# raznem/spp-rl

Measured on AMD Instinct MI355X. Metric: env-steps/sec (rollout+update) SPP-SAC Hopper-v2, higher is better.
Workload: dtype fp32

## Files before the change

### spp-rl_amd/csrc/common.h

```cpp
#pragma once
#include <hip/hip_runtime.h>
#include <stdint.h>

#include <string>

#ifndef SPP_BF16_TWO_TILES
#define SPP_BF16_TWO_TILES 0
#endif
#ifndef SPP_BF16_FUSE3
#define SPP_BF16_FUSE3 0
#endif

typedef float f32x16 __attribute__((ext_vector_type(16)));
typedef float f32x4 __attribute__((ext_vector_type(4)));

namespace spp {

constexpr int kWave = 64;
constexpr int kTile = 32;
constexpr int kHidden = 256;

void set_error(const char* fmt, ...);
const char* get_error();

#define SPP_CHECK_HIP(expr)                                                        \
  do {                                                                             \
    hipError_t e_ = (expr);                                                        \
    if (e_ != hipSuccess) {                                                        \
      ::spp::set_error("%s:%d %s -> %s", __FILE__, __LINE__, #expr, hipGetErrorString(e_)); \
      return SPP_E_HIP;                                                            \
    }                                                                              \
  } while (0)

#define SPP_REQUIRE(cond, code, ...)        \
  do {                                      \
    if (!(cond)) {                          \
      ::spp::set_error(__VA_ARGS__);        \
      return code;                          \
    }                                       \
  } while (0)

inline int64_t round_up(int64_t x, int64_t m) { return (x + m - 1) / m * m; }
inline int cdiv(int64_t x, int64_t m) { return (int)((x + m - 1) / m); }
// ... 82 lines not shown
```

### spp-rl_amd/csrc/mlp.h

```cpp
#pragma once
#include "common.h"

namespace spp {
#define SPP_XLANE_SYNC() asm volatile("" ::: "memory")


#ifdef SPP_PROF
__device__ unsigned long long g_tprof[64];
__shared__ unsigned long long s_tprof[4][32];
__shared__ unsigned long long s_tlast[4];
#ifdef SPP_PROF_DRAIN
#define SPP_TP_DRAIN() asm volatile("s_waitcnt vmcnt(0) lgkmcnt(0)" ::: "memory")
#else
#define SPP_TP_DRAIN()
#endif
#define SPP_TP_INIT()                                                            \
  {                                                                              \
    const int w_ = threadIdx.x >> 6;                                             \
    if ((threadIdx.x & 63) < 32 && w_ < 4) s_tprof[w_][threadIdx.x & 63] = 0;    \
    if ((threadIdx.x & 63) == 0 && w_ < 4) s_tlast[w_] = clock64();              \
  }
#define SPP_TP(k)                                                                \
  {                                                                              \
    __builtin_amdgcn_sched_barrier(0);                                           \
// ... 133 lines not shown
  for (int b = 0; b < NBI; ++b) {
    if (q < base + rv_get(RV, b)) return q - base;
    base += rv_get(RV, b);
  }
  return 0;
}

__device__ __forceinline__ constexpr int ru(int r) { return (r & 3) + 8 * (r >> 2); }

__device__ __forceinline__ f32x16 bias_tile(const float* biasL, int ob, int h) {
  f32x16 acc;
  const float4* b4 = reinterpret_cast<const float4*>(biasL + 32 * ob + 4 * h);
#pragma unroll
  for (int k = 0; k < 4; ++k) {
    const float4 v = b4[2 * k];
    acc[4 * k + 0] = v.x;
    acc[4 * k + 1] = v.y;
    acc[4 * k + 2] = v.z;
    acc[4 * k + 3] = v.w;
  }
  return acc;
}

typedef __amdgpu_buffer_rsrc_t rsrc_t;
__device__ __forceinline__ rsrc_t rsrc_n(const void* p, int nbytes) {
  return __builtin_amdgcn_make_buffer_rsrc(const_cast<void*>(p), (short)0, nbytes, 0x00020000);
}
__device__ __forceinline__ rsrc_t rsrc(const void* p) { return rsrc_n(p, 0x7fffffff); }
__device__ __forceinline__ float4 wfrag(rsrc_t w, uint32_t lane16, int off) {
  asm volatile("" : "+s"(off));
  return __builtin_bit_cast(float4, __builtin_amdgcn_raw_buffer_load_b128(w, lane16, off, 0));
}

template <int NBI, uint64_t RV, bool BIAS, typename Epi>
__device__ __forceinline__ void dense_impl(const float4* __restrict__ Wf, int NBO, const f32x16 (&in)[NBI],
                                           const float* biasL, Epi&& epi) {
  constexpr int NQ = rv_total(RV, NBI);
  static_assert(NQ > 0, "empty layer");
  constexpr int CH = chunk_of(NQ);
  constexpr int NC = NQ / CH;
  static_assert(NQ % CH == 0, "chunking");
  const int lane = lane_id();
  const int h = lane >> 5;
  const rsrc_t wr = rsrc(Wf);
  const uint32_t l16 = 16u * lane;
  constexpr int OBSTRIDE = NBI * 4 * 64 * 16;
  float4 cur[CH];
  static_for<0, CH>([&](auto I) {
    constexpr int q = decltype(I)::value;
    cur[q] = wfrag(wr, l16, (q_ib(RV, NBI, q) * 4 + q_rq(RV, NBI, q)) * 1024);
  });
  auto chain = [&](int ob) {
    f32x16 acc;
    if constexpr (BIAS) acc = bias_tile(biasL, ob, h);
    else acc = zero16();
    const int obn = ob + 1 < NBO ? ob + 1 : ob;
    static_for<0, NC>([&](auto C) {
      constexpr int c = decltype(C)::value;
      constexpr int nc = (c + 1 < NC) ? c + 1 : 0;
      const int wn = ((c + 1 < NC) ? ob : obn) * OBSTRIDE;
      float4 nxt[CH];
      static_for<0, CH>([&](auto I) {
        constexpr int q = nc * CH + decltype(I)::value;
        nxt[decltype(I)::value] = wfrag(wr, l16, wn + (q_ib(RV, NBI, q) * 4 + q_rq(RV, NBI, q)) * 1024);
      });
      static_for<0, CH>([&](auto I) {
        constexpr int i = decltype(I)::value;
        constexpr int q = c * CH + i;
        constexpr int ib = q_ib(RV, NBI, q);
        constexpr int rq = q_rq(RV, NBI, q);
        acc = mfma(cur[i].x, in[ib][4 * rq + 0], acc);
        acc = mfma(cur[i].y, in[ib][4 * rq + 1], acc);
        acc = mfma(cur[i].z, in[ib][4 * rq + 2], acc);
        acc = mfma(cur[i].w, in[ib][4 * rq + 3], acc);
      });
#pragma unroll
      for (int i = 0; i < CH; ++i) cur[i] = nxt[i];
    });
    return acc;
  };
  SPP_TPD(23);
  f32x16 prev = chain(0);
#pragma unroll 1
  for (int ob = 1; ob < NBO; ++ob) {
    const f32x16 acc = chain(ob);
    epi(ob - 1, prev);
    prev = acc;
  }
  SPP_TPD(24);
  epi(NBO - 1, prev);
  SPP_TPD(25);
}

constexpr int cgcd(int a, int b) { return b ? cgcd(b, a % b) : a; }

template <int NBO, bool BIAS, typename Epi>
__device__ __forceinline__ void dense_lds_impl(const float4* __restrict__ Wf, const float* img, const float* biasL,
                                               Epi&& epi) {
  constexpr int NQ = NBO * 4;
  constexpr int CH = 4;
  constexpr int NCI = NQ / CH;
  constexpr int D = 4;
  constexpr int U = NCI * D / cgcd(NCI, D);
  constexpr int IBU = U / NCI;
  constexpr int G = 8 * NCI;
  static_assert(8 % IBU == 0, "input blocks per iteration");
  constexpr int NIT = 8 / IBU;
  const int lane = lane_id();
  const int h = lane >> 5;
  const float* l = img + 4 * h * 32 + (lane & 31);
  const rsrc_t wr = rsrc(Wf);
  const uint32_t l16 = 16u * lane;
  f32x16 acc[NBO];
  static_for<0, NBO>([&](auto O) {
    if constexpr (BIAS) acc[O] = bias_tile(biasL, O, h);
    else acc[O] = zero16();
  });
  float4 ring[D][CH];
  static_for<0, D - 1>([&](auto I) {
    static_for<0, CH>([&](auto J) { ring[I][J] = wfrag(wr, l16, ((int)I * CH + (int)J) * 1024); });
  });
  f32x16 xin[IBU];
  static_for<0, IBU>([&](auto K) {
// ... 45 lines not shown
  return __builtin_amdgcn_mfma_f32_32x32x16_bf16(a, b, c, 0, 0, 0);
}
__device__ __forceinline__ bf16x8 frag16(float4 v) { return __builtin_bit_cast(bf16x8, v); }
template <int S>
__device__ __forceinline__ bf16x8 to_bf16x8(const f32x16& t) {
  bf16x8 r;
#pragma unroll
  for (int j = 0; j < 8; ++j) r[j] = (__bf16)t[8 * S + j];
  return r;
}
constexpr int st_get(uint64_t RV, int ib) { return (rv_get(RV, ib) + 1) / 2; }
constexpr int st_total(uint64_t RV, int nb) {
  int t = 0;
  for (int ib = 0; ib < nb; ++ib) t += st_get(RV, ib);
  return t;
}
constexpr int st_ib(uint64_t RV, int NBI, int q) {
  int base = 0;
  for (int b = 0; b < NBI; ++b) {
    if (q < base + st_get(RV, b)) return b;
    base += st_get(RV, b);
  }
  return NBI - 1;
}
constexpr int st_s(uint64_t RV, int NBI, int q) {
  int base = 0;
  for (int b = 0; b < NBI; ++b) {
    if (q < base + st_get(RV, b)) return q - base;
    base += st_get(RV, b);
  }
  return 0;
}

template <int NBI, uint64_t RV, bool BIAS, typename Epi>
__device__ __forceinline__ void dense16_impl(const float4* __restrict__ Wf, int NBO, const f32x16 (&in)[NBI],
                                             const float* biasL, Epi&& epi) {
  constexpr int NS = st_total(RV, NBI);
  static_assert(NS > 0, "empty layer");
  const int lane = lane_id();
  const int h = lane >> 5;
  const rsrc_t wr = rsrc(Wf);
  const uint32_t l16 = 16u * lane;
  constexpr int OBSTRIDE = NBI * 2 * 64 * 16;
  bf16x8 bin[NS];
  static_for<0, NS>([&](auto Q) {
    constexpr int q = Q;
    bin[q] = to_bf16x8<st_s(RV, NBI, q)>(in[st_ib(RV, NBI, q)]);
  });
  float4 cur[NS];
  static_for<0, NS>([&](auto Q) {
    constexpr int q = Q;
    cur[q] = wfrag(wr, l16, (st_ib(RV, NBI, q) * 2 + st_s(RV, NBI, q)) * 1024);
  });
  auto chain = [&](int ob) {
    f32x16 acc;
    if constexpr (BIAS) acc = bias_tile(biasL, ob, h);
    else acc = zero16();
    const int wn = (ob + 1 < NBO ? ob + 1 : ob) * OBSTRIDE;
    float4 nxt[NS];
    static_for<0, NS>([&](auto Q) {
      constexpr int q = Q;
      nxt[q] = wfrag(wr, l16, wn + (st_ib(RV, NBI, q) * 2 + st_s(RV, NBI, q)) * 1024);
    });
    static_for<0, NS>([&](auto Q) { acc = mfma16(frag16(cur[(int)Q]), bin[(int)Q], acc); });
#pragma unroll
    for (int q = 0; q < NS; ++q) cur[q] = nxt[q];
    return acc;
  };
  f32x16 prev = chain(0);
#pragma unroll 1
  for (int ob = 1; ob < NBO; ++ob) {
    const f32x16 acc = chain(ob);
    epi(ob - 1, prev);
    prev = acc;
  }
  epi(NBO - 1, prev);
}

template <int NBO, bool BIAS, typename Epi>
__device__ __forceinline__ void dense16_lds_impl(const float4* __restrict__ Wf, const float* img, const float* biasL,
                                                 Epi&& epi) {
  const int lane = lane_id();
  const int h = lane >> 5;
  const float* l = img + 4 * h * 32 + (lane & 31);
  const rsrc_t wr = rsrc(Wf);
  const uint32_t l16 = 16u * lane;
  f32x16 acc[NBO];
  static_for<0, NBO>([&](auto O) {
    if constexpr (BIAS) acc[O] = bias_tile(biasL, O, h);
    else acc[O] = zero16();
  });
  float4 fr[2][2 * NBO];
  static_for<0, 2 * NBO>([&](auto J) { fr[0][J] = wfrag(wr, l16, (int)J * 1024); });
  f32x16 x;
#pragma unroll
  for (int r = 0; r < 16; ++r) x[r] = l[ru(r) * 32];
  static_for<0, 8>([&](auto IB) {
    constexpr int ib = IB;
    const bf16x8 b0 = to_bf16x8<0>(x), b1 = to_bf16x8<1>(x);
    if constexpr (ib + 1 < 8) {
      static_for<0, 2 * NBO>([&](auto J) {
        fr[(ib + 1) & 1][J] = wfrag(wr, l16, ((ib + 1) * NBO * 2 + (int)J) * 1024);
      });
    }
    __builtin_amdgcn_sched_barrier(0);
    static_for<0, NBO>([&](auto O) {
      constexpr int ob = O;
      acc[ob] = mfma16(frag16(fr[ib & 1][2 * ob]), b0, acc[ob]);
      acc[ob] = mfma16(frag16(fr[ib & 1][2 * ob + 1]), b1, acc[ob]);
    });
    if constexpr (ib + 1 < 8) {
#pragma unroll
      for (int r = 0; r < 16; ++r) x[r] = l[(32 * (ib + 1) + ru(r)) * 32];
    }
  });
  static_for<0, NBO>([&](auto O) { epi(IC<(int)O>{}, acc[O]); });
}

template <int NBI, uint64_t RV, bool BF = false, typename Epi>
__device__ __forceinline__ void dense(const float4* __restrict__ Wf, int NBO, const f32x16 (&in)[NBI],
                                      const float* biasL, Epi&& epi) {
  if constexpr (BF) dense16_impl<NBI, RV, true>(Wf, NBO, in, biasL, static_cast<Epi&&>(epi));
  else dense_impl<NBI, RV, true>(Wf, NBO, in, biasL, static_cast<Epi&&>(epi));
}
template <int NBI, uint64_t RV, bool BF = false, typename Epi>
__device__ __forceinline__ void dense(const float4* __restrict__ Wf, int NBO, const f32x16 (&in)[NBI], decltype(nullptr),
                                      Epi&& epi) {
  if constexpr (BF) dense16_impl<NBI, RV, false>(Wf, NBO, in, nullptr, static_cast<Epi&&>(epi));
  else dense_impl<NBI, RV, false>(Wf, NBO, in, nullptr, static_cast<Epi&&>(epi));
}
template <int NBO, bool BF = false, typename Epi>
__device__ __forceinline__ void dense_lds(const float4* __restrict__ Wf, const float* img, const float* biasL,
                                          Epi&& epi) {
  if constexpr (BF) dense16_lds_impl<NBO, true>(Wf, img, biasL, static_cast<Epi&&>(epi));
  else dense_lds_impl<NBO, true>(Wf, img, biasL, static_cast<Epi&&>(epi));
}
template <int NBO, bool BF = false, typename Epi>
__device__ __forceinline__ void dense_lds(const float4* __restrict__ Wf, const float* img, decltype(nullptr),
                                          Epi&& epi) {
  if constexpr (BF) dense16_lds_impl<NBO, false>(Wf, img, nullptr, static_cast<Epi&&>(epi));
  else dense_lds_impl<NBO, false>(Wf, img, nullptr, static_cast<Epi&&>(epi));
}


#ifndef SPP_OPST_AUX
#define SPP_OPST_AUX 2
#endif
#ifndef SPP_STREAM_LD_AUX
#define SPP_STREAM_LD_AUX 0
#endif

__device__ __forceinline__ int lane_off(int ld, int b) { return 4 * (lane_id() >> 5) * ld + b; }

template <int NB>
__device__ __forceinline__ void lds_load(f32x16 (&t)[NB], const float* lds) {
  const int lane = lane_id();
  const float* l = lds + 4 * (lane >> 5) * 32 + (lane & 31);
#pragma unroll
  for (int ib = 0; ib < NB; ++ib)
#pragma unroll
    for (int r = 0; r < 16; ++r) t[ib][r] = l[(32 * ib + ru(r)) * 32];
}
// ... 57 lines not shown
```

### spp-rl_amd/csrc/sac.hip

```cpp
#pragma once
#include "sac_kernels.h"

namespace spp {

constexpr float kLog2 = 0.69314718055994530942f;
constexpr float kLogSqrt2Pi = 0.91893853320467274178f;

template <int OB_, int AOUT_, int AC_, bool ACMC_, bool BF_ = false>
struct Cfg {
  static constexpr int OB = OB_, AOUT = AOUT_, AC = AC_;
  static constexpr bool ACMC = ACMC_;
  static constexpr bool BF = BF_;
  static constexpr bool F3 = !BF_ || SPP_BF16_FUSE3;
  static constexpr int NB_OB = blocks_of(OB);
  static constexpr int NB_AOUT = blocks_of(AOUT);
  static constexpr int NB_H2 = blocks_of(2 * AOUT);
  static constexpr int NB_PAIR = (AOUT + 15) / 16;
  static constexpr int CA = ACMC ? AC : AOUT;
  static constexpr int NB_CA = blocks_of(CA);
  static constexpr int NB_CIN = NB_OB + NB_CA;
  static constexpr int NB_ACMIN = NB_OB + NB_AOUT;
  static constexpr uint64_t RV_X = rv_nat(OB, NB_OB);
  static constexpr uint64_t RV_H = rv_nat(256, 8);
  static constexpr uint64_t RV_CIN = rv_cat(OB, NB_OB, CA, NB_CA);
  static constexpr uint64_t RV_ACMIN = rv_cat(OB, NB_OB, AOUT, NB_AOUT);
  static constexpr uint64_t RV_Z1 = rv_nat(64, 2);
  static constexpr uint64_t RV_Z2 = rv_nat(32, 1);
  static constexpr uint64_t RV_AC = rv_nat(AC, 1);
  static constexpr uint64_t RV_CA = rv_nat(CA, NB_CA);
  static constexpr uint64_t RV_PAIR = rv_pair(AOUT, NB_PAIR);
  static_assert(AC <= 32, "env action dim <= 32");
  static_assert(2 * AOUT <= 256 && OB + AOUT <= 256, "dims");
};

constexpr int kWavesPerWG = 4;

constexpr int kLdsPerWave = 256 * 32;
constexpr int kSmallRow = 192;

__device__ __forceinline__ void load_table(const SacArgs& p, float* tbl) {
  for (int s = 0; s < p.nseg; ++s) {
    const TabSeg g = p.seg[s];
    for (int i = threadIdx.x; i < g.npad; i += blockDim.x) tbl[g.off + i] = i < g.n ? g.src[i] : 0.f;
  }
  __syncthreads();
}
__device__ __forceinline__ float tval(const float* t, int ob, int q, int h4) { return t[32 * ob + ru(q) + h4]; }
__device__ __forceinline__ void tvals(const float* t, int ob, int h4, float (&v)[16]) {
  const float4* p = reinterpret_cast<const float4*>(t + 32 * ob + h4);
#pragma unroll
  for (int k = 0; k < 4; ++k) {
    const float4 x = p[2 * k];
    v[4 * k + 0] = x.x;
    v[4 * k + 1] = x.y;
    v[4 * k + 2] = x.z;
    v[4 * k + 3] = x.w;
  }
}

__device__ __forceinline__ void setbits(uint64_t& lo, uint64_t& hi, int ob, uint32_t bits) {
  if (ob < 4) lo |= (uint64_t)bits << (16 * ob);
  else hi |= (uint64_t)bits << (16 * (ob - 4));
  asm volatile("" : "+v"(lo), "+v"(hi));
}
__device__ __forceinline__ bool getbit(uint64_t lo, uint64_t hi, int ob, int q) {
  const uint64_t w = ob < 4 ? (lo >> (16 * ob)) : (hi >> (16 * (ob - 4)));
// ... 121 lines not shown
  uint32_t vo, vp;
  float *bl, *sl;
  float* pl;
};
__device__ __forceinline__ Lane make_lane(float* big, float* small, const float* tbl, int ld, int b) {
  Lane L;
  L.img = big;
  L.tbl = tbl;
  int lane = lane_id();
  asm volatile("" : "+v"(lane));
  int ld4 = 4 * ld;
  asm volatile("" : "+s"(ld4));
  L.h = lane >> 5;
  L.s = lane & 31;
  L.h4 = 4 * L.h;
  L.ld4 = ld4;
  L.b = b;
  L.vo = (uint32_t)(L.h4 * ld4 + 4 * b);
  L.vp = (uint32_t)(8 * L.h * ld4 + 4 * b);
  L.bl = big + L.h4 * 32 + L.s;
  L.sl = small + L.h4 * 32 + L.s;
  L.pl = big + 8 * L.h * 32 + L.s;
  return L;
}

template <class C, bool ST, int NBH = C::NB_H2, int NHR = 2 * C::AOUT>
__device__ __forceinline__ void actor_trunk(const ActorDev& A, const float* X, int xbytes, const Lane& L, float* H1g,
                                            float* H2g,
                                            uint64_t& m1lo, uint64_t& m1hi, uint64_t& m2lo, uint64_t& m2hi) {
  {
    f32x16 x[C::NB_OB];
    gm_load<C::NB_OB>(x, X, xbytes, C::OB, L.ld4, L.vo);
    const rsrc_t hr = rsrc(H1g);
    dense<C::NB_OB, C::RV_X, C::BF>(A.W1, 8, x, L.tbl + A.tb1, [&](int ob, const f32x16& acc) {
      uint32_t bits = 0;
#pragma unroll
      for (int q = 0; q < 16; ++q) {
        const int ur = 32 * ob + ru(q);
        const float v = fmaxf(acc[q], 0.f);
        L.bl[ur * 32] = v;
        if constexpr (ST) op_st<C::BF>(hr, ur, L.ld4, L.vo, v);
        bits |= (uint32_t)(v > 0.f) << q;
      }
      setbits(m1lo, m1hi, ob, bits);
    });
  }
  SPP_TP(1);
  {
    const rsrc_t hr = rsrc(H2g);
    dense_lds<8, C::BF>(A.W2, L.img, L.tbl + A.tb2, [&](int ob, const f32x16& acc) {
      uint32_t bits = 0;
#pragma unroll
      for (int q = 0; q < 16; ++q) {
        const int ur = 32 * ob + ru(q);
        const float v = fmaxf(acc[q], 0.f);
        L.bl[ur * 32] = v;
        if constexpr (ST) op_st<C::BF>(hr, ur, L.ld4, L.vo, v);
        bits |= (uint32_t)(v > 0.f) << q;
      }
      setbits(m2lo, m2hi, ob, bits);
    });
  }
  SPP_TP(2);
  {
    dense_lds<NBH, C::BF>(A.Wh, L.img, L.tbl + A.tbh, [&](int ob, const f32x16& acc) {
#pragma unroll
      for (int q = 0; q < 16; ++q) {
        const int ur = 32 * ob + ru(q);
        if (ur + L.h4 < NHR) L.bl[ur * 32] = acc[q];
      }
    });
  }
  SPP_TP(3);
}

template <class C, bool ST>
__device__ __forceinline__ void acm_forward(const SacArgs& p, const f32x16 (&xin)[C::NB_ACMIN], const Lane& L,
                                            float* Z1g, float* Z2g, float* T3g) {
  float* small = L.sl - L.h4 * 32 - L.s;
  const rsrc_t z1r = rsrc(Z1g), z2r = rsrc(Z2g), t3r = rsrc(T3g);
  dense<C::NB_ACMIN, C::RV_ACMIN, C::BF>(p.acm.W1, 2, xin, L.tbl + p.acm.tb1, [&](int ob, const f32x16& acc) {
#pragma unroll
    for (int q = 0; q < 16; ++q) {
      const int ur = 32 * ob + ru(q);
      const float v = tanhf(acc[q]);
      L.sl[ur * 32] = v;
      if constexpr (ST) fm_st(z1r, ur, L.ld4, L.vo, v);
    }
  });
  f32x16 z1[2];
  lds_load<2>(z1, small);
  dense<2, C::RV_Z1, C::BF>(p.acm.W2, 1, z1, L.tbl + p.acm.tb2, [&](int ob, const f32x16& acc) {
#pragma unroll
    for (int q = 0; q < 16; ++q) {
      const float v = tanhf(acc[q]);
      L.sl[ru(q) * 32] = v;
      if constexpr (ST) fm_st(z2r, ru(q), L.ld4, L.vo, v);
    }
  });
  f32x16 z2[1];
  lds_load<1>(z2, small);
  float limv[16];
#pragma unroll
  for (int q = 0; q < 16; ++q) {
    const int u = ru(q) + L.h4;
    limv[q] = acm_lim<true>(p, L.tbl, u < C::AC ? u : 0);
  }
  dense<1, C::RV_Z2, C::BF>(p.acm.W3, 1, z2, L.tbl + p.acm.tb3, [&](int ob, const f32x16& acc) {
#pragma unroll
    for (int q = 0; q < 16; ++q) {
      const int u = ru(q) + L.h4;
      if (u < C::AC) {
        const float t = tanhf(acc[q]);
        L.sl[ru(q) * 32] = t * limv[q];
        if constexpr (ST) fm_st(t3r, ru(q), L.ld4, L.vo, t);
      }
    }
  });
}

template <class C, bool ST, int R = 30, bool H2L = false>
__device__ __forceinline__ float critic_forward(const CriticDev& Q, const f32x16 (&xin)[C::NB_CIN], const Lane& L,
                                                float* H1g, float* H2g, uint64_t& m1lo, uint64_t& m1hi,
                                                uint64_t& m2lo, uint64_t& m2hi) {
  const rsrc_t h1r = rsrc(H1g), h2r = rsrc(H2g);
  dense<C::NB_CIN, C::RV_CIN, C::BF>(Q.W1, 8, xin, L.tbl + Q.tb1, [&](int ob, const f32x16& acc) {
    uint32_t bits = 0;
#pragma unroll
    for (int q = 0; q < 16; ++q) {
      const int ur = 32 * ob + ru(q);
      const float v = fmaxf(acc[q], 0.f);
      L.bl[ur * 32] = v;
      if constexpr (ST) op_st<C::BF>(h1r, ur, L.ld4, L.vo, v);
      bits |= (uint32_t)(v > 0.f) << q;
    }
    setbits(m1lo, m1hi, ob, bits);
  });
  SPP_TP(R);
  float qp = 0.f;
  const float* w3 = L.tbl + Q.tw3;
  dense_lds<8, C::BF>(Q.W2, L.img, L.tbl + Q.tb2, [&](int ob, const f32x16& acc) {
    uint32_t bits = 0;
    float tv[16];
    tvals(w3, ob, L.h4, tv);
#pragma unroll
    for (int q = 0; q < 16; ++q) {
      const float v = fmaxf(acc[q], 0.f);
      if constexpr (H2L) L.bl[(32 * ob + ru(q)) * 32] = v;
      else if constexpr (ST) op_st<C::BF>(h2r, 32 * ob + ru(q), L.ld4, L.vo, v);
      qp = fmaf(v, tv[q], qp);
      bits |= (uint32_t)(v > 0.f) << q;
    }
    setbits(m2lo, m2hi, ob, bits);
  });
  SPP_TP(R + 1);
  return qp + __shfl_xor(qp, 32, 64) + *Q.b3;
}

template <class C, bool BRF = false>
// ... 148 lines not shown
      });
    }
    SPP_TP(14);
    const float s0 = wave_sum(lq0), s1 = wave_sum(lq1);
    if (lane == 0) {
      p.part[tile * kParts + 0] = s0;
      p.part[tile * kParts + 1] = s1;
    }
    SPP_TP(15);
  }
  if constexpr (C::F3) {
    const int64_t wg = (int64_t)blockIdx.x * kWavesPerWG + w;
    float* o0 = p.W3P[0] + wg * p.w3p_stride;
    float* o1 = p.W3P[1] + wg * p.w3p_stride;
#pragma unroll
    for (int k = 0; k < 4; ++k) {
      o0[lane + 64 * k] = w3a[k];
      o1[lane + 64 * k] = w3b[k];
    }
    if (lane == 0) {
      o0[256] = b3a;
      o1[256] = b3b;
    }
  }
  SPP_TP_FLUSH();
}

struct AcmScratch {
  float *Z1, *Z2, *T3;
  float* GAD;
  uint64_t* MASK;
};

template <class C>
__global__ __launch_bounds__(256, 1) void k_sac_actor_phase(SacArgs p, AcmScratch z) {
  __shared__ float smem[kWavesPerWG * kLdsPerWave];
  __shared__ __attribute__((aligned(16))) float tbl[kTabMax];
  SPP_TP_INIT();
  load_table(p, tbl);
  const int w = threadIdx.x >> 6, lane = threadIdx.x & 63;
  float* big = smem + w * kLdsPerWave;
  float* small = big + kSmallRow * 32;
  const int ntiles = p.Bp / 32;
  const int ld = p.Bp;
  const float alpha = *p.alpha;
  for (int tile = blockIdx.x * kWavesPerWG + w; tile < ntiles; tile += gridDim.x * kWavesPerWG) {
    const Lane L = make_lane(big, small, tbl, ld, tile * 32 + (lane & 31));
    const int b = L.b;
    const bool valid = b < p.B;
    const float g_lp = valid ? alpha * p.inv_B : 0.f;
    uint64_t a1lo = 0, a1hi = 0, a2lo = 0, a2hi = 0;
    SPP_TP(26);
    actor_trunk<C, true>(p.actor, p.S, C::OB * L.ld4, L, p.AH1, p.AH2, a1lo, a1hi, a2lo, a2hi);
    SPP_TP(27);
    f32x16 hd[C::NB_PAIR];
    load_pair<C>(hd, big);
    const float lp = squash_write<C>(p, hd, p.EPS2, L);
    SPP_TP(28);
    constexpr bool kParkHeads = C::NB_PAIR > 2;
    if constexpr (kParkHeads) {
#pragma unroll
      for (int ib = 0; ib < C::NB_PAIR; ++ib)
#pragma unroll
        for (int r = 0; r < 8; ++r) {
          const int j0 = 16 * ib + r;
          if (j0 + 8 * L.h < C::AOUT) {
            fm_st(rsrc(p.ADH), j0, L.ld4, L.vp, hd[ib][r]);
            fm_st(rsrc(p.ADH), C::AOUT + j0, L.ld4, L.vp, hd[ib][r + 8]);
// ... 52 lines not shown
      constexpr bool kPre = !kParkHeads;
      float t3v[16], limv[16], z2v[16], z1v[2][16];
      const rsrc_t t3r = rsrc_n(z.T3, C::AC * L.ld4);
#pragma unroll
      for (int q = 0; q < 16; ++q) {
        const int u = ru(q) + L.h4;
        t3v[q] = fm_ldb(t3r, ru(q), L.ld4, L.vo);
        limv[q] = acm_lim<true>(p, L.tbl, u < C::AC ? u : 0);
      }
      if constexpr (kPre) {
#pragma unroll
        for (int q = 0; q < 16; ++q) z2v[q] = fm_ld(rsrc(z.Z2), ru(q), L.ld4, L.vo);
#pragma unroll
        for (int ob = 0; ob < 2; ++ob)
#pragma unroll
          for (int q = 0; q < 16; ++q) z1v[ob][q] = fm_ld(rsrc(z.Z1), 32 * ob + ru(q), L.ld4, L.vo);
      }
      auto z2at = [&](int q) {
        if constexpr (kPre) return z2v[q];
        else return fm_ld(rsrc(z.Z2), ru(q), L.ld4, L.vo);
      };
      auto z1at = [&](int ob, int q) {
        if constexpr (kPre) return ob ? z1v[1][q] : z1v[0][q];
        else return fm_ld(rsrc(z.Z1), 32 * ob + ru(q), L.ld4, L.vo);
      };
      f32x16 dp3[1];
#pragma unroll
      for (int q = 0; q < 16; ++q) {
        const int u = ru(q) + L.h4;
        const float t = t3v[q];
        dp3[0][q] = u < C::AC ? dca[0][q] * limv[q] * (1.f - t * t) : 0.f;
      }
      SPP_TPN(23);
      dense<1, C::RV_AC, C::BF>(p.acm.W3T, 1, dp3, nullptr, [&](int ob, const f32x16& acc) {
#pragma unroll
        for (int q = 0; q < 16; ++q) {
          const float zz = z2at(q);
          L.sl[ru(q) * 32] = acc[q] * (1.f - zz * zz);
        }
      });
      SPP_TPN(24);
      f32x16 dp2[1];
      lds_load<1>(dp2, small);
      dense<1, C::RV_Z2, C::BF>(p.acm.W2T, 2, dp2, nullptr, [&](int ob, const f32x16& acc) {
#pragma unroll
        for (int q = 0; q < 16; ++q) {
          const float zz = z1at(ob, q);
          L.sl[(32 * ob + ru(q)) * 32] = acc[q] * (1.f - zz * zz);
        }
      });
      SPP_TPN(25);
      f32x16 dp1[2];
      lds_load<2>(dp1, small);
      dense<2, C::RV_Z1, C::BF>(p.acm.W1Ta, C::NB_AOUT, dp1, nullptr, [&](int ob, const f32x16& acc) {
#pragma unroll
        for (int q = 0; q < 16; ++q) {
          const int ur = 32 * ob + ru(q);
          if (ur + L.h4 < C::AOUT) L.bl[ur * 32] = acc[q];
        }
      });
    } else {
#pragma unroll
      for (int ib = 0; ib < C::NB_CA; ++ib)
#pragma unroll
        for (int q = 0; q < 16; ++q) {
          const int ur = 32 * ib + ru(q);
          if (ur + L.h4 < C::AOUT) L.bl[ur * 32] = dca[ib][q];
        }
    }
    SPP_TP(16);
    if constexpr (kParkHeads) {
      const rsrc_t gr = rsrc(z.GAD);
#pragma unroll
      for (int ib = 0; ib < C::NB_AOUT; ++ib)
#pragma unroll
        for (int q = 0; q < 16; ++q) {
          const int ur = 32 * ib + ru(q);
          if (ur + L.h4 < C::AOUT) fm_st(gr, ur, L.ld4, L.vo, L.bl[ur * 32]);
        }
      uint64_t* mk = z.MASK + (int64_t)tile * 4 * 64 + lane;
      mk[0] = a1lo;
      mk[64] = a1hi;
      mk[128] = a2lo;
      mk[192] = a2hi;
      const float ps = wave_sum((valid && L.h == 0) ? fsub_rn(alpha * lp, qmin) : 0.f);
      const float pl = wave_sum((valid && L.h == 0) ? lp : 0.f);
      if (lane == 0) {
// ... 36 lines not shown
          if (closs) {
            if (p.norm_closs) {
              const float df = fsub_rn(a, normalize<true>(p, L.tbl, jj, s2));
              g_a += cl_scale * df;
              dist_part += (valid && ok) ? df * df : 0.f;
            } else {
              const float df = fsub_rn(denorm<true>(p, L.tbl, jj, a), s2);
              g_ad += cl_scale * df;
              dist_part += (valid && ok) ? df * df : 0.f;
            }
          }
          g_a += g_ad * denorm_scale<true>(p, L.tbl, jj);
          const float var = fmul_rn(sc, sc);
          const float sig_m2u = 1.f / (1.f + expf(2.f * u));
          const float gu = g_a * lim * (1.f - t * t) + g_lp * (-d / var + 2.f - 4.f * sig_m2u);
          const float gmu = gu + g_lp * d / var;
          const float gsc = gu * e + g_lp * (d * d / (var * sc) - 1.f / sc);
          const float gls = (lsr >= -20.f && lsr <= 2.f) ? gsc * sc : 0.f;
          hd[ib][r] = ok ? gmu : 0.f;
          hd[ib][r + 8] = ok ? gls : 0.f;
        }
  #pragma unroll
      for (int ib = 0; ib < C::NB_PAIR; ++ib)
  #pragma unroll
        for (int r = 0; r < 8; ++r) {
          const int j0 = 16 * ib + r;
          if (j0 + h8 < C::AOUT) {
            fm_st(rsrc(p.ADH), j0, L.ld4, L.vp, hd[ib][r]);
            fm_st(rsrc(p.ADH), C::AOUT + j0, L.ld4, L.vp, hd[ib][r + 8]);
          }
        }
    }
    SPP_TP(17);
    dense<C::NB_PAIR, C::RV_PAIR, C::BF>(p.actor.WhT, 8, hd, nullptr, [&](int ob, const f32x16& acc) {
#pragma unroll
      for (int q = 0; q < 16; ++q) {
        const int ur = 32 * ob + ru(q);
        const float v = getbit(a2lo, a2hi, ob, q) ? acc[q] : 0.f;
        L.bl[ur * 32] = v;
        op_st<C::BF>(rsrc(p.AD2), ur, L.ld4, L.vo, v);
      }
    });
    {
      dense_lds<8, C::BF>(p.actor.W2T, big, nullptr, [&](int ob, const f32x16& acc) {
#pragma unroll
        for (int q = 0; q < 16; ++q)
          op_st<C::BF>(rsrc(p.AD1), 32 * ob + ru(q), L.ld4, L.vo, getbit(a1lo, a1hi, ob, q) ? acc[q] : 0.f);
      });
    }
    SPP_TP(18);
    const float ps = wave_sum(sac_part);
    const float pd = wave_sum(dist_part);
    const float pl = wave_sum((valid && L.h == 0) ? lp : 0.f);
    if (lane == 0) {
      p.part[tile * kParts + 2] = ps;
      p.part[tile * kParts + 3] = pd;
      p.part[tile * kParts + 4] = pl;
    }
  }
  SPP_TP_FLUSH();
}

template <class C>
__global__ __launch_bounds__(256, 1) void k_sac_actor_heads(SacArgs p, AcmScratch z) {
  __shared__ float smem[kWavesPerWG * kLdsPerWave];
  __shared__ __attribute__((aligned(16))) float tbl[kTabMax];
  SPP_TP_INIT();
// ... 55 lines not shown
          } else {
            const float df = fsub_rn(denorm<true>(p, L.tbl, jj, a), s2v[r]);
            g_ad += cl_scale * df;
            dist_part += (valid && ok) ? df * df : 0.f;
          }
        }
        g_a += g_ad * denorm_scale<true>(p, L.tbl, jj);
        const float var = fmul_rn(sc, sc);
        const float ivar = t_rcp<F>(var), isc = t_rcp<F>(sc);
        const float sig_m2u = t_rcp<F>(1.f + t_exp<F>(2.f * u));
        const float gu = g_a * lim * (1.f - t * t) + g_lp * (-d * ivar + 2.f - 4.f * sig_m2u);
        const float gmu = gu + g_lp * d * ivar;
        const float gsc = gu * e + g_lp * (d * d * ivar * isc - isc);
        const float gls = (lsr[r] >= -20.f && lsr[r] <= 2.f) ? gsc * sc : 0.f;
        if (ok) {
          L.pl[j0 * 32] = gmu;
          L.pl[(C::AOUT + j0) * 32] = gls;
        }
      }
    }
    f32x16 hd[C::NB_PAIR];
    load_pair<C>(hd, big);
#pragma unroll
    for (int ib = 0; ib < C::NB_PAIR; ++ib)
#pragma unroll
      for (int r = 0; r < 8; ++r) {
        const int j0 = 16 * ib + r;
        if (j0 + h8 < C::AOUT) {
          fm_st(rsrc(p.ADH), j0, L.ld4, L.vp, hd[ib][r]);
          fm_st(rsrc(p.ADH), C::AOUT + j0, L.ld4, L.vp, hd[ib][r + 8]);
        }
      }
    SPP_TP(17);
    dense<C::NB_PAIR, C::RV_PAIR, C::BF>(p.actor.WhT, 8, hd, nullptr, [&](int ob, const f32x16& acc) {
#pragma unroll
      for (int q = 0; q < 16; ++q) {
        const int ur = 32 * ob + ru(q);
        const float v = getbit(a2lo, a2hi, ob, q) ? acc[q] : 0.f;
        L.bl[ur * 32] = v;
        op_st<C::BF>(rsrc(p.AD2), ur, L.ld4, L.vo, v);
      }
    });
    dense_lds<8, C::BF>(p.actor.W2T, big, nullptr, [&](int ob, const f32x16& acc) {
#pragma unroll
      for (int q = 0; q < 16; ++q)
        op_st<C::BF>(rsrc(p.AD1), 32 * ob + ru(q), L.ld4, L.vo, getbit(a1lo, a1hi, ob, q) ? acc[q] : 0.f);
    });
    SPP_TP(18);
    const float pd = wave_sum(dist_part);
    if (lane == 0) p.part[tile * kParts + 3] = pd;
  }
  SPP_TP_FLUSH();
}

struct ActArgs {
  int E, mode, denorm_out;
  float act_noise;
  const float *obs, *eps, *noise;
  float *target_out, *env_out;
  int plain;
};

template <class C>
__global__ __launch_bounds__(256, 1) void k_policy_act(SacArgs p, ActArgs a) {
  __shared__ float smem[kWavesPerWG * kLdsPerWave];
  __shared__ __attribute__((aligned(16))) float tbl[kTabMax];
  load_table(p, tbl);
// ... 76 lines not shown
__global__ __launch_bounds__(256, 1) void k_acm_regress(SacArgs p, AcmRegArgs g) {
  __shared__ float smem[kWavesPerWG * kLdsPerWave];
  __shared__ __attribute__((aligned(16))) float tbl[kTabMax];
  load_table(p, tbl);
  const int w = threadIdx.x >> 6, lane = threadIdx.x & 63;
  float* big = smem + w * kLdsPerWave;
  float* small = big + kSmallRow * 32;
  const int ntiles = g.Bp / 32;
  const int ld = g.Bp;
  constexpr int IN = 2 * C::OB;
  constexpr int NB_IN = blocks_of(IN);
  constexpr uint64_t RV_IN = rv_nat(IN, NB_IN);
  for (int tile = blockIdx.x * kWavesPerWG + w; tile < ntiles; tile += gridDim.x * kWavesPerWG) {
    const Lane L = make_lane(big, small, tbl, ld, tile * 32 + (lane & 31));
    const int b = L.b;
    const bool valid = b < g.B;
    const int br = valid ? b : 0;
    f32x16 xin[NB_IN];
#pragma unroll
    for (int ib = 0; ib < NB_IN; ++ib)
#pragma unroll
      for (int r = 0; r < 16; ++r) {
        const int ur = 32 * ib + ru(r);
        const int u = ur + L.h4;
        xin[ib][r] = (u < IN && valid) ? g.x[br * IN + u] : 0.f;
      }
#pragma unroll
    for (int ib = 0; ib < NB_IN; ++ib)
#pragma unroll
      for (int r = 0; r < 16; ++r) {
        const int ur = 32 * ib + ru(r);
        if (ur + L.h4 < IN) fm_st(rsrc(g.XT), ur, L.ld4, L.vo, xin[ib][r]);
      }
    dense<NB_IN, RV_IN, C::BF>(p.acm.W1, 2, xin, tbl + p.acm.tb1, [&](int ob, const f32x16& acc) {
#pragma unroll
      for (int q = 0; q < 16; ++q) {
        const int ur = 32 * ob + ru(q);
        const float v = tanhf(acc[q]);
        L.sl[ur * 32] = v;
        fm_st(rsrc(g.Z1), ur, L.ld4, L.vo, v);
      }
    });
    f32x16 z1[2];
    lds_load<2>(z1, small);
    dense<2, C::RV_Z1, C::BF>(p.acm.W2, 1, z1, tbl + p.acm.tb2, [&](int ob, const f32x16& acc) {
#pragma unroll
      for (int q = 0; q < 16; ++q) {
        const float v = tanhf(acc[q]);
        L.sl[ru(q) * 32] = v;
        fm_st(rsrc(g.Z2), ru(q), L.ld4, L.vo, v);
      }
    });
    f32x16 z2[1];
    lds_load<1>(z2, small);
    float lsum = 0.f;
    f32x16 p3[1];
    const float sc = 2.f / ((float)g.B * (float)C::AC);
    float limv[16], yv[16];
#pragma unroll
    for (int q = 0; q < 16; ++q) {
      const int u = ru(q) + L.h4;
      const int uu = u < C::AC ? u : 0;
      limv[q] = acm_lim<true>(p, L.tbl, uu);
      yv[q] = g.y[br * C::AC + uu];
    }
    dense<1, C::RV_Z2, C::BF>(p.acm.W3, 1, z2, tbl + p.acm.tb3, [&](int ob, const f32x16& acc) {
#pragma unroll
      for (int q = 0; q < 16; ++q) {
        const int u = ru(q) + L.h4;
        float v = 0.f;
        if (u < C::AC && valid) {
          const float t = tanhf(acc[q]);
          const float lim = limv[q];
          const float df = fsub_rn(fmul_rn(t, lim), yv[q]);
          lsum += df * df;
          v = sc * df * lim * (1.f - t * t);
        }
        p3[0][q] = v;
        if (u < C::AC) fm_st(rsrc(g.P3), ru(q), L.ld4, L.vo, v);
      }
    });
    dense<1, C::RV_AC, C::BF>(p.acm.W3T, 1, p3, nullptr, [&](int ob, const f32x16& acc) {
#pragma unroll
      for (int q = 0; q < 16; ++q) {
        const float zz = z2[0][q];
        const float v = acc[q] * (1.f - zz * zz);
        L.sl[ru(q) * 32] = v;
        fm_st(rsrc(g.P2), ru(q), L.ld4, L.vo, v);
      }
    });
    f32x16 p2[1];
    lds_load<1>(p2, small);
    dense<1, C::RV_Z2, C::BF>(p.acm.W2T, 2, p2, nullptr, [&](int ob, const f32x16& acc) {
#pragma unroll
      for (int q = 0; q < 16; ++q) {
        const int ur = 32 * ob + ru(q);
        const float zz = ob == 0 ? z1[0][q] : z1[1][q];
        fm_st(rsrc(g.P1), ur, L.ld4, L.vo, acc[q] * (1.f - zz * zz));
      }
    });
    const float ls = wave_sum(lsum);
    if (lane == 0) g.part[tile] = ls;
  }
}

#ifndef SPP_KSET_TU
struct StageArgs {
  int B, Bp, ob, aout, ac;
  const float *obs, *next_obs, *act, *rew, *acm;
  const int8_t* done;
  const float *eps1, *eps2;
  float *S, *S2, *ACT, *AENV, *R, *DN, *EPS1, *EPS2;
};
__global__ void k_stage_batch(StageArgs a) {
  const int64_t b = (int64_t)blockIdx.x * blockDim.x + threadIdx.x;
  if (b >= a.Bp) return;
  const bool v = b < a.B;
  const int64_t ld = a.Bp;
  for (int f = 0; f < a.ob; ++f) {
    a.S[f * ld + b] = v ? a.obs[b * a.ob + f] : 0.f;
    a.S2[f * ld + b] = v ? a.next_obs[b * a.ob + f] : 0.f;
  }
  for (int f = 0; f < a.aout; ++f) {
    if (a.act) a.ACT[f * ld + b] = v ? a.act[b * a.aout + f] : 0.f;
    if (a.eps1) a.EPS1[f * ld + b] = v ? a.eps1[b * a.aout + f] : 0.f;
    if (a.eps2) a.EPS2[f * ld + b] = v ? a.eps2[b * a.aout + f] : 0.f;
// ... 83 lines not shown
```

Before: 421,700.

## Software-pipeline dense layer output blocks, interleaving MFMA chains with epilogues

```diff
diff --git a/spp-rl_amd/csrc/common.h b/spp-rl_amd/csrc/common.h
--- a/spp-rl_amd/csrc/common.h
+++ b/spp-rl_amd/csrc/common.h
@@ -9,6 +9,12 @@
 #endif
 #ifndef SPP_BF16_FUSE3
 #define SPP_BF16_FUSE3 0
+#endif
+#ifndef SPP_DENSE_PIPE
+#define SPP_DENSE_PIPE 1
+#endif
+#ifndef SPP_DENSE16_PIPE
+#define SPP_DENSE16_PIPE 0
 #endif
 
 typedef float f32x16 __attribute__((ext_vector_type(16)));
diff --git a/spp-rl_amd/csrc/mlp.h b/spp-rl_amd/csrc/mlp.h
--- a/spp-rl_amd/csrc/mlp.h
+++ b/spp-rl_amd/csrc/mlp.h
@@ -189,7 +189,63 @@
   return __builtin_bit_cast(float4, __builtin_amdgcn_raw_buffer_load_b128(w, lane16, off, 0));
 }
 
-template <int NBI, uint64_t RV, bool BIAS, typename Epi>
+template <int NM>
+__device__ __forceinline__ void sched_chain_epi() {
+  constexpr int NV = (104 + NM - 1) / NM, NW = (16 + NM - 1) / NM;
+  static_for<0, NM>([&](auto I) {
+    if constexpr (decltype(I)::value > 0) __builtin_amdgcn_sched_group_barrier(0x008, 1, 0);
+    __builtin_amdgcn_sched_group_barrier(0x040, NW, 0);
+    __builtin_amdgcn_sched_group_barrier(0x200, NW, 0);
+    __builtin_amdgcn_sched_group_barrier(0x002, NV, 0);
+  });
+}
+
+template <bool PIPE, int NM, typename Chain, typename Bias, typename Epi>
+__device__ __forceinline__ void dense_blocks(int NBO, Chain&& chain, Bias&& bias, Epi&& epi) {
+  if constexpr (PIPE) {
+    auto slot = [&](auto NB, int ob, f32x16& acc, const f32x16& done, f32x16& nxt, int obn) {
+      __builtin_amdgcn_sched_barrier(0);
+      acc = chain(ob, [&] { return acc; }, [] { __builtin_amdgcn_sched_barrier(0); });
+      if constexpr (decltype(NB)::value) nxt = bias(obn);
+      f32x16 t = done;
+      asm("" : "+v"(t));
+      epi(ob - 1, t);
+      sched_chain_epi<NM>();
+      __builtin_amdgcn_sched_barrier(0);
+    };
+    f32x16 t0 = chain(0, [&] { return bias(0); }, [] {}), t1 = bias(NBO > 1 ? 1 : 0), t2;
+    int ob = 1;
+#pragma unroll 1
+    for (; ob + 2 < NBO; ob += 3) {
+      slot(IC<1>{}, ob, t1, t0, t2, ob + 1);
+      slot(IC<1>{}, ob + 1, t2, t1, t0, ob + 2);
+      slot(IC<1>{}, ob + 2, t0, t2, t1, ob + 3 < NBO ? ob + 3 : ob + 2);
+    }
+    SPP_TPD(24);
+    if (ob + 1 < NBO) {
+      slot(IC<1>{}, ob, t1, t0, t2, ob + 1);
+      slot(IC<0>{}, ob + 1, t2, t1, t0, 0);
+      epi(ob + 1, t2);
+    } else if (ob < NBO) {
+      slot(IC<0>{}, ob, t1, t0, t2, 0);
+      epi(ob, t1);
+    } else {
+      epi(NBO - 1, t0);
+    }
+  } else {
+    f32x16 prev = chain(0, [&] { return bias(0); }, [] {});
+#pragma unroll 1
+    for (int ob = 1; ob < NBO; ++ob) {
+      const f32x16 acc = chain(ob, [&] { return bias(ob); }, [] {});
+      epi(ob - 1, prev);
+      prev = acc;
+    }
+    SPP_TPD(24);
+    epi(NBO - 1, prev);
+  }
+}
+
+template <int NBI, uint64_t RV, bool BIAS, bool PIPE, typename Epi>
 __device__ __forceinline__ void dense_impl(const float4* __restrict__ Wf, int NBO, const f32x16 (&in)[NBI],
                                            const float* biasL, Epi&& epi) {
   constexpr int NQ = rv_total(RV, NBI);
@@ -207,9 +263,9 @@
     constexpr int q = decltype(I)::value;
     cur[q] = wfrag(wr, l16, (q_ib(RV, NBI, q) * 4 + q_rq(RV, NBI, q)) * 1024);
   });
-  auto chain = [&](int ob) {
+  auto chain = [&](int ob, auto&& c0, auto&& mid) {
     f32x16 acc;
-    if constexpr (BIAS) acc = bias_tile(biasL, ob, h);
+    if constexpr (BIAS) acc = c0();
     else acc = zero16();
     const int obn = ob + 1 < NBO ? ob + 1 : ob;
     static_for<0, NC>([&](auto C) {
@@ -227,6 +283,7 @@
         constexpr int ib = q_ib(RV, NBI, q);
         constexpr int rq = q_rq(RV, NBI, q);
         acc = mfma(cur[i].x, in[ib][4 * rq + 0], acc);
+        if constexpr (q == 0) mid();
         acc = mfma(cur[i].y, in[ib][4 * rq + 1], acc);
         acc = mfma(cur[i].z, in[ib][4 * rq + 2], acc);
         acc = mfma(cur[i].w, in[ib][4 * rq + 3], acc);
@@ -236,16 +293,53 @@
     });
     return acc;
   };
+  auto bias = [&](int ob) {
+    if constexpr (BIAS) return bias_tile(biasL, ob, h);
+    else return zero16();
+  };
   SPP_TPD(23);
-  f32x16 prev = chain(0);
+  if constexpr (PIPE) {
+    dense_blocks<true, 4 * NQ>(NBO, chain, bias, static_cast<Epi&&>(epi));
+  } else {
+    auto chain1 = [&](int ob) {
+      f32x16 acc;
+      if constexpr (BIAS) acc = bias_tile(biasL, ob, h);
+      else acc = zero16();
+      const int obn = ob + 1 < NBO ? ob + 1 : ob;
+      static_for<0, NC>([&](auto C) {
+        constexpr int c = decltype(C)::value;
+        constexpr int nc = (c + 1 < NC) ? c + 1 : 0;
+        const int wn = ((c + 1 < NC) ? ob : obn) * OBSTRIDE;
+        float4 nxt[CH];
+        static_for<0, CH>([&](auto I) {
+          constexpr int q = nc * CH + decltype(I)::value;
+          nxt[decltype(I)::value] = wfrag(wr, l16, wn + (q_ib(RV, NBI, q) * 4 + q_rq(RV, NBI, q)) * 1024);
+        });
+        static_for<0, CH>([&](auto I) {
+          constexpr int i = decltype(I)::value;
+          constexpr int q = c * CH + i;
+          constexpr int ib = q_ib(RV, NBI, q);
+          constexpr int rq = q_rq(RV, NBI, q);
+          acc = mfma(cur[i].x, in[ib][4 * rq + 0], acc);
+          acc = mfma(cur[i].y, in[ib][4 * rq + 1], acc);
+          acc = mfma(cur[i].z, in[ib][4 * rq + 2], acc);
+          acc = mfma(cur[i].w, in[ib][4 * rq + 3], acc);
+        });
+#pragma unroll
+        for (int i = 0; i < CH; ++i) cur[i] = nxt[i];
+      });
+      return acc;
+    };
+    f32x16 prev = chain1(0);
 #pragma unroll 1
-  for (int ob = 1; ob < NBO; ++ob) {
-    const f32x16 acc = chain(ob);
-    epi(ob - 1, prev);
-    prev = acc;
-  }
-  SPP_TPD(24);
-  epi(NBO - 1, prev);
+    for (int ob = 1; ob < NBO; ++ob) {
+      const f32x16 acc = chain1(ob);
+      epi(ob - 1, prev);
+      prev = acc;
+    }
+    SPP_TPD(24);
+    epi(NBO - 1, prev);
+  }
   SPP_TPD(25);
 }
 
@@ -357,7 +451,7 @@
   return 0;
 }
 
-template <int NBI, uint64_t RV, bool BIAS, typename Epi>
+template <int NBI, uint64_t RV, bool BIAS, bool PIPE, typename Epi>
 __device__ __forceinline__ void dense16_impl(const float4* __restrict__ Wf, int NBO, const f32x16 (&in)[NBI],
                                              const float* biasL, Epi&& epi) {
   constexpr int NS = st_total(RV, NBI);
@@ -377,9 +471,9 @@
     constexpr int q = Q;
     cur[q] = wfrag(wr, l16, (st_ib(RV, NBI, q) * 2 + st_s(RV, NBI, q)) * 1024);
   });
-  auto chain = [&](int ob) {
+  auto chain = [&](int ob, auto&& c0, auto&& mid) {
     f32x16 acc;
-    if constexpr (BIAS) acc = bias_tile(biasL, ob, h);
+    if constexpr (BIAS) acc = c0();
     else acc = zero16();
     const int wn = (ob + 1 < NBO ? ob + 1 : ob) * OBSTRIDE;
     float4 nxt[NS];
@@ -387,19 +481,19 @@
       constexpr int q = Q;
       nxt[q] = wfrag(wr, l16, wn + (st_ib(RV, NBI, q) * 2 + st_s(RV, NBI, q)) * 1024);
     });
-    static_for<0, NS>([&](auto Q) { acc = mfma16(frag16(cur[(int)Q]), bin[(int)Q], acc); });
+    static_for<0, NS>([&](auto Q) {
+      acc = mfma16(frag16(cur[(int)Q]), bin[(int)Q], acc);
+      if constexpr (decltype(Q)::value == 0) mid();
+    });
 #pragma unroll
     for (int q = 0; q < NS; ++q) cur[q] = nxt[q];
     return acc;
   };
-  f32x16 prev = chain(0);
-#pragma unroll 1
-  for (int ob = 1; ob < NBO; ++ob) {
-    const f32x16 acc = chain(ob);
-    epi(ob - 1, prev);
-    prev = acc;
-  }
-  epi(NBO - 1, prev);
+  auto bias = [&](int ob) {
+    if constexpr (BIAS) return bias_tile(biasL, ob, h);
+    else return zero16();
+  };
+  dense_blocks<PIPE, NS>(NBO, chain, bias, static_cast<Epi&&>(epi));
 }
 
 template <int NBO, bool BIAS, typename Epi>
@@ -442,17 +536,18 @@
   static_for<0, NBO>([&](auto O) { epi(IC<(int)O>{}, acc[O]); });
 }
 
-template <int NBI, uint64_t RV, bool BF = false, typename Epi>
+constexpr bool dense_pipe_default(bool bf) { return (bf ? SPP_DENSE16_PIPE : SPP_DENSE_PIPE) != 0; }
+template <int NBI, uint64_t RV, bool BF = false, bool PIPE = dense_pipe_default(BF), typename Epi>
 __device__ __forceinline__ void dense(const float4* __restrict__ Wf, int NBO, const f32x16 (&in)[NBI],
                                       const float* biasL, Epi&& epi) {
-  if constexpr (BF) dense16_impl<NBI, RV, true>(Wf, NBO, in, biasL, static_cast<Epi&&>(epi));
-  else dense_impl<NBI, RV, true>(Wf, NBO, in, biasL, static_cast<Epi&&>(epi));
-}
-template <int NBI, uint64_t RV, bool BF = false, typename Epi>
+  if constexpr (BF) dense16_impl<NBI, RV, true, PIPE>(Wf, NBO, in, biasL, static_cast<Epi&&>(epi));
+  else dense_impl<NBI, RV, true, PIPE>(Wf, NBO, in, biasL, static_cast<Epi&&>(epi));
+}
+template <int NBI, uint64_t RV, bool BF = false, bool PIPE = dense_pipe_default(BF), typename Epi>
 __device__ __forceinline__ void dense(const float4* __restrict__ Wf, int NBO, const f32x16 (&in)[NBI], decltype(nullptr),
                                       Epi&& epi) {
-  if constexpr (BF) dense16_impl<NBI, RV, false>(Wf, NBO, in, nullptr, static_cast<Epi&&>(epi));
-  else dense_impl<NBI, RV, false>(Wf, NBO, in, nullptr, static_cast<Epi&&>(epi));
+  if constexpr (BF) dense16_impl<NBI, RV, false, PIPE>(Wf, NBO, in, nullptr, static_cast<Epi&&>(epi));
+  else dense_impl<NBI, RV, false, PIPE>(Wf, NBO, in, nullptr, static_cast<Epi&&>(epi));
 }
 template <int NBO, bool BF = false, typename Epi>
 __device__ __forceinline__ void dense_lds(const float4* __restrict__ Wf, const float* img, const float* biasL,
diff --git a/spp-rl_amd/csrc/sac.hip b/spp-rl_amd/csrc/sac.hip
--- a/spp-rl_amd/csrc/sac.hip
+++ b/spp-rl_amd/csrc/sac.hip
@@ -12,6 +12,7 @@
   static constexpr bool ACMC = ACMC_;
   static constexpr bool BF = BF_;
   static constexpr bool F3 = !BF_ || SPP_BF16_FUSE3;
+  static constexpr bool PIPE = dense_pipe_default(BF_);
   static constexpr int NB_OB = blocks_of(OB);
   static constexpr int NB_AOUT = blocks_of(AOUT);
   static constexpr int NB_H2 = blocks_of(2 * AOUT);
@@ -32,6 +33,15 @@
   static_assert(AC <= 32, "env action dim <= 32");
   static_assert(2 * AOUT <= 256 && OB + AOUT <= 256, "dims");
 };
+
+template <class C>
+struct NoPipe : C {
+  static constexpr bool PIPE = false;
+};
+template <class C>
+constexpr bool actor_phase_pipe() {
+  return C::OB < 17 || (C::OB == 17 && C::AOUT == 17 && !C::ACMC);
+}
 
 constexpr int kWavesPerWG = 4;
 
@@ -219,7 +229,7 @@
     f32x16 x[C::NB_OB];
     gm_load<C::NB_OB>(x, X, xbytes, C::OB, L.ld4, L.vo);
     const rsrc_t hr = rsrc(H1g);
-    dense<C::NB_OB, C::RV_X, C::BF>(A.W1, 8, x, L.tbl + A.tb1, [&](int ob, const f32x16& acc) {
+    dense<C::NB_OB, C::RV_X, C::BF, C::PIPE>(A.W1, 8, x, L.tbl + A.tb1, [&](int ob, const f32x16& acc) {
       uint32_t bits = 0;
 #pragma unroll
       for (int q = 0; q < 16; ++q) {
@@ -266,7 +276,7 @@
                                             float* Z1g, float* Z2g, float* T3g) {
   float* small = L.sl - L.h4 * 32 - L.s;
   const rsrc_t z1r = rsrc(Z1g), z2r = rsrc(Z2g), t3r = rsrc(T3g);
-  dense<C::NB_ACMIN, C::RV_ACMIN, C::BF>(p.acm.W1, 2, xin, L.tbl + p.acm.tb1, [&](int ob, const f32x16& acc) {
+  dense<C::NB_ACMIN, C::RV_ACMIN, C::BF, C::PIPE>(p.acm.W1, 2, xin, L.tbl + p.acm.tb1, [&](int ob, const f32x16& acc) {
 #pragma unroll
     for (int q = 0; q < 16; ++q) {
       const int ur = 32 * ob + ru(q);
@@ -277,7 +287,7 @@
   });
   f32x16 z1[2];
   lds_load<2>(z1, small);
-  dense<2, C::RV_Z1, C::BF>(p.acm.W2, 1, z1, L.tbl + p.acm.tb2, [&](int ob, const f32x16& acc) {
+  dense<2, C::RV_Z1, C::BF, C::PIPE>(p.acm.W2, 1, z1, L.tbl + p.acm.tb2, [&](int ob, const f32x16& acc) {
 #pragma unroll
     for (int q = 0; q < 16; ++q) {
       const float v = tanhf(acc[q]);
@@ -293,7 +303,7 @@
     const int u = ru(q) + L.h4;
     limv[q] = acm_lim<true>(p, L.tbl, u < C::AC ? u : 0);
   }
-  dense<1, C::RV_Z2, C::BF>(p.acm.W3, 1, z2, L.tbl + p.acm.tb3, [&](int ob, const f32x16& acc) {
+  dense<1, C::RV_Z2, C::BF, C::PIPE>(p.acm.W3, 1, z2, L.tbl + p.acm.tb3, [&](int ob, const f32x16& acc) {
 #pragma unroll
     for (int q = 0; q < 16; ++q) {
       const int u = ru(q) + L.h4;
@@ -311,7 +321,7 @@
                                                 float* H1g, float* H2g, uint64_t& m1lo, uint64_t& m1hi,
                                                 uint64_t& m2lo, uint64_t& m2hi) {
   const rsrc_t h1r = rsrc(H1g), h2r = rsrc(H2g);
-  dense<C::NB_CIN, C::RV_CIN, C::BF>(Q.W1, 8, xin, L.tbl + Q.tb1, [&](int ob, const f32x16& acc) {
+  dense<C::NB_CIN, C::RV_CIN, C::BF, C::PIPE>(Q.W1, 8, xin, L.tbl + Q.tb1, [&](int ob, const f32x16& acc) {
     uint32_t bits = 0;
 #pragma unroll
     for (int q = 0; q < 16; ++q) {
@@ -526,8 +536,9 @@
   uint64_t* MASK;
 };
 
-template <class C>
+template <class C0>
 __global__ __launch_bounds__(256, 1) void k_sac_actor_phase(SacArgs p, AcmScratch z) {
+  using C = std::conditional_t<actor_phase_pipe<C0>(), C0, NoPipe<C0>>;
   __shared__ float smem[kWavesPerWG * kLdsPerWave];
   __shared__ __attribute__((aligned(16))) float tbl[kTabMax];
   SPP_TP_INIT();
@@ -646,7 +657,7 @@
         dp3[0][q] = u < C::AC ? dca[0][q] * limv[q] * (1.f - t * t) : 0.f;
       }
       SPP_TPN(23);
-      dense<1, C::RV_AC, C::BF>(p.acm.W3T, 1, dp3, nullptr, [&](int ob, const f32x16& acc) {
+      dense<1, C::RV_AC, C::BF, C::PIPE>(p.acm.W3T, 1, dp3, nullptr, [&](int ob, const f32x16& acc) {
 #pragma unroll
         for (int q = 0; q < 16; ++q) {
           const float zz = z2at(q);
@@ -656,7 +667,7 @@
       SPP_TPN(24);
       f32x16 dp2[1];
       lds_load<1>(dp2, small);
-      dense<1, C::RV_Z2, C::BF>(p.acm.W2T, 2, dp2, nullptr, [&](int ob, const f32x16& acc) {
+      dense<1, C::RV_Z2, C::BF, C::PIPE>(p.acm.W2T, 2, dp2, nullptr, [&](int ob, const f32x16& acc) {
 #pragma unroll
         for (int q = 0; q < 16; ++q) {
           const float zz = z1at(ob, q);
@@ -666,7 +677,7 @@
       SPP_TPN(25);
       f32x16 dp1[2];
       lds_load<2>(dp1, small);
-      dense<2, C::RV_Z1, C::BF>(p.acm.W1Ta, C::NB_AOUT, dp1, nullptr, [&](int ob, const f32x16& acc) {
+      dense<2, C::RV_Z1, C::BF, C::PIPE>(p.acm.W1Ta, C::NB_AOUT, dp1, nullptr, [&](int ob, const f32x16& acc) {
 #pragma unroll
         for (int q = 0; q < 16; ++q) {
           const int ur = 32 * ob + ru(q);
@@ -769,7 +780,7 @@
         }
     }
     SPP_TP(17);
-    dense<C::NB_PAIR, C::RV_PAIR, C::BF>(p.actor.WhT, 8, hd, nullptr, [&](int ob, const f32x16& acc) {
+    dense<C::NB_PAIR, C::RV_PAIR, C::BF, C::PIPE>(p.actor.WhT, 8, hd, nullptr, [&](int ob, const f32x16& acc) {
 #pragma unroll
       for (int q = 0; q < 16; ++q) {
         const int ur = 32 * ob + ru(q);
@@ -891,7 +902,7 @@
         }
       }
     SPP_TP(17);
-    dense<C::NB_PAIR, C::RV_PAIR, C::BF>(p.actor.WhT, 8, hd, nullptr, [&](int ob, const f32x16& acc) {
+    dense<C::NB_PAIR, C::RV_PAIR, C::BF, C::PIPE>(p.actor.WhT, 8, hd, nullptr, [&](int ob, const f32x16& acc) {
 #pragma unroll
       for (int q = 0; q < 16; ++q) {
         const int ur = 32 * ob + ru(q);
@@ -1034,7 +1045,7 @@
         const int ur = 32 * ib + ru(r);
         if (ur + L.h4 < IN) fm_st(rsrc(g.XT), ur, L.ld4, L.vo, xin[ib][r]);
       }
-    dense<NB_IN, RV_IN, C::BF>(p.acm.W1, 2, xin, tbl + p.acm.tb1, [&](int ob, const f32x16& acc) {
+    dense<NB_IN, RV_IN, C::BF, C::PIPE>(p.acm.W1, 2, xin, tbl + p.acm.tb1, [&](int ob, const f32x16& acc) {
 #pragma unroll
       for (int q = 0; q < 16; ++q) {
         const int ur = 32 * ob + ru(q);
@@ -1045,7 +1056,7 @@
     });
     f32x16 z1[2];
     lds_load<2>(z1, small);
-    dense<2, C::RV_Z1, C::BF>(p.acm.W2, 1, z1, tbl + p.acm.tb2, [&](int ob, const f32x16& acc) {
+    dense<2, C::RV_Z1, C::BF, C::PIPE>(p.acm.W2, 1, z1, tbl + p.acm.tb2, [&](int ob, const f32x16& acc) {
 #pragma unroll
       for (int q = 0; q < 16; ++q) {
         const float v = tanhf(acc[q]);
@@ -1066,7 +1077,7 @@
       limv[q] = acm_lim<true>(p, L.tbl, uu);
       yv[q] = g.y[br * C::AC + uu];
     }
-    dense<1, C::RV_Z2, C::BF>(p.acm.W3, 1, z2, tbl + p.acm.tb3, [&](int ob, const f32x16& acc) {
+    dense<1, C::RV_Z2, C::BF, C::PIPE>(p.acm.W3, 1, z2, tbl + p.acm.tb3, [&](int ob, const f32x16& acc) {
 #pragma unroll
       for (int q = 0; q < 16; ++q) {
         const int u = ru(q) + L.h4;
@@ -1082,7 +1093,7 @@
         if (u < C::AC) fm_st(rsrc(g.P3), ru(q), L.ld4, L.vo, v);
       }
     });
-    dense<1, C::RV_AC, C::BF>(p.acm.W3T, 1, p3, nullptr, [&](int ob, const f32x16& acc) {
+    dense<1, C::RV_AC, C::BF, C::PIPE>(p.acm.W3T, 1, p3, nullptr, [&](int ob, const f32x16& acc) {
 #pragma unroll
       for (int q = 0; q < 16; ++q) {
         const float zz = z2[0][q];
@@ -1093,7 +1104,7 @@
     });
     f32x16 p2[1];
     lds_load<1>(p2, small);
-    dense<1, C::RV_Z2, C::BF>(p.acm.W2T, 2, p2, nullptr, [&](int ob, const f32x16& acc) {
+    dense<1, C::RV_Z2, C::BF, C::PIPE>(p.acm.W2T, 2, p2, nullptr, [&](int ob, const f32x16& acc) {
 #pragma unroll
       for (int q = 0; q < 16; ++q) {
         const int ur = 32 * ob + ru(q);
```

After: 424,000, median of 6. About the same (+0.5%).
